# GEO-IASS/bn-pp

Hardware: NVIDIA B200
Metric: factor entries/sec (fused product+sum-out), VE PR on 2^28-entry tables (higher is better)
Workload: dtype f64

## Files before the change

### bnpp_b200/capi.py

```python
import ctypes
import os

_HERE = os.path.dirname(os.path.abspath(__file__))
LIB_PATH = os.path.join(_HERE, "libbnpp_b200.so")

c_u32p = ctypes.POINTER(ctypes.c_uint32)
c_i32p = ctypes.POINTER(ctypes.c_int32)
c_i64p = ctypes.POINTER(ctypes.c_int64)
c_u64p = ctypes.POINTER(ctypes.c_uint64)
c_f64p = ctypes.POINTER(ctypes.c_double)

EXPORTS = [
    "bnpp_version", "bnpp_ctx_create", "bnpp_ctx_destroy", "bnpp_ctx_sync", "bnpp_ctx_status", "bnpp_last_error",
    "bnpp_launch_count", "bnpp_last_launch", "bnpp_alloc", "bnpp_free", "bnpp_upload", "bnpp_download", "bnpp_fill",
    "bnpp_union_scope", "bnpp_scope_size", "bnpp_product_sum_out", "bnpp_product", "bnpp_sum_out", "bnpp_condition",
    "bnpp_normalize", "bnpp_reduce", "bnpp_fg_create", "bnpp_fg_destroy", "bnpp_fg_sweep", "bnpp_fg_update",
    "bnpp_fg_marginals", "bnpp_elim_order", "bnpp_order_width", "bnpp_ve_plan_create", "bnpp_ve_plan_destroy",
    "bnpp_ve_plan_info", "bnpp_ve_plan_run", "bnpp_ve_plan_run_batched", "bnpp_ve_plan_set_profiling",
    "bnpp_ve_plan_step_stats", "bnpp_ve_plan_step_kernel", "bnpp_ve_plan_set_fused", "bnpp_ve_plan_fused_info", "bnpp_ve_plan_fused_program", "bnpp_ve_plan_describe", "bnpp_ve_plan_set_segments", "bnpp_ve_plan_segments", "bnpp_ve_plan_segment_program", "bnpp_mar_plan_create", "bnpp_mar_plan_layout", "bnpp_pick_shard_vars",
    "bnpp_tuning_set", "bnpp_tuning_get", "bnpp_ve_plan_result_size", "bnpp_ve_plan_set_normalize",
    "bnpp_mar_plan_normalize", "bnpp_fg_reset", "bnpp_ve_plan_launches",
    "bnpp_sampler_create", "bnpp_sampler_destroy", "bnpp_sampler_logical", "bnpp_sampler_likelihood",
    "bnpp_product_max_out", "bnpp_mpe_plan_create", "bnpp_mpe_plan_run", "bnpp_mpe_plan_run_batched",
    "bnpp_elim_order_constrained", "bnpp_map_plan_create", "bnpp_mpe_plan_nvars", "bnpp_mpe_shard_select",
    "bnpp_ve_plan_windows",
]


def tuning_set(key, value):
    L = lib()
    L.bnpp_tuning_set.argtypes = [ctypes.c_char_p, ctypes.c_uint64]
    L.bnpp_tuning_get.argtypes = [ctypes.c_char_p, c_u64p]
    old = ctypes.c_uint64()
    if L.bnpp_tuning_get(key.encode(), ctypes.byref(old)) != 0 or L.bnpp_tuning_set(key.encode(), int(value)) != 0:
        raise BnppError(-1, "unknown tuning key %r" % key)
    return old.value


class Scope(ctypes.Structure):
    _fields_ = [("rank", ctypes.c_int32), ("var_id", c_u32p), ("card", c_u32p)]


class Operand(ctypes.Structure):
    _fields_ = [("data", ctypes.c_void_p), ("scope", Scope), ("stride", c_i64p)]


class BnppError(RuntimeError):
    def __init__(self, code, msg):
        super().__init__("bnpp_b200 error %d: %s" % (code, msg))
        self.code = code


_lib = None


def lib():
    global _lib
    if _lib is None:
        if not os.path.exists(LIB_PATH):
            raise RuntimeError("bnpp_b200: %s is not built (run `python -c 'import __graft_entry__ as g; g.build()'`); "
                               "there is no CPU fallback" % LIB_PATH)
        L = ctypes.CDLL(LIB_PATH)
        L.bnpp_last_error.restype = ctypes.c_char_p
        L.bnpp_last_error.argtypes = [ctypes.c_void_p]
        L.bnpp_launch_count.restype = ctypes.c_uint64
        L.bnpp_launch_count.argtypes = [ctypes.c_void_p]
        L.bnpp_scope_size.restype = ctypes.c_uint64
        L.bnpp_ctx_create.argtypes = [ctypes.c_int, ctypes.c_void_p, ctypes.POINTER(ctypes.c_void_p)]
        L.bnpp_ctx_destroy.argtypes = [ctypes.c_void_p]
        L.bnpp_ctx_sync.argtypes = [ctypes.c_void_p]
        L.bnpp_ctx_status.argtypes = [ctypes.c_void_p, c_u32p, ctypes.c_int]
        L.bnpp_last_launch.argtypes = [ctypes.c_void_p, ctypes.c_char_p, ctypes.c_size_t, c_u32p, c_u32p]
        L.bnpp_alloc.argtypes = [ctypes.c_void_p, ctypes.c_uint64, ctypes.POINTER(ctypes.c_void_p)]
        L.bnpp_free.argtypes = [ctypes.c_void_p, ctypes.c_void_p]
        L.bnpp_upload.argtypes = [ctypes.c_void_p, ctypes.c_void_p, ctypes.c_void_p, ctypes.c_uint64]
        L.bnpp_download.argtypes = [ctypes.c_void_p, ctypes.c_void_p, ctypes.c_void_p, ctypes.c_uint64]
        L.bnpp_fill.argtypes = [ctypes.c_void_p, ctypes.c_void_p, ctypes.c_uint64, ctypes.c_double]
        L.bnpp_union_scope.argtypes = [ctypes.POINTER(Scope), ctypes.POINTER(Scope), c_u32p, c_u32p]
        L.bnpp_scope_size.argtypes = [ctypes.POINTER(Scope)]
        L.bnpp_product_sum_out.argtypes = [ctypes.c_void_p, ctypes.c_int, ctypes.POINTER(Operand), ctypes.POINTER(Scope),
                                           ctypes.c_int64, ctypes.c_int, ctypes.c_void_p, ctypes.c_void_p]
        L.bnpp_product_max_out.argtypes = [ctypes.c_void_p, ctypes.c_int, ctypes.POINTER(Operand), ctypes.POINTER(Scope),
                                           ctypes.c_int64, ctypes.c_void_p, ctypes.c_void_p]
        L.bnpp_product.argtypes = [ctypes.c_void_p, ctypes.POINTER(Scope), ctypes.c_void_p, ctypes.POINTER(Scope),
                                   ctypes.c_void_p, ctypes.c_int, ctypes.c_void_p, ctypes.c_void_p]
        L.bnpp_sum_out.argtypes = [ctypes.c_void_p, ctypes.POINTER(Scope), ctypes.c_void_p, ctypes.c_uint32,
                                   ctypes.c_void_p, ctypes.c_void_p]
        L.bnpp_condition.argtypes = [ctypes.c_void_p, ctypes.POINTER(Scope), ctypes.c_void_p, ctypes.c_int, c_u32p, c_u32p,
                                     ctypes.c_void_p, ctypes.c_void_p]
        L.bnpp_normalize.argtypes = [ctypes.c_void_p, ctypes.c_uint64, ctypes.c_void_p, ctypes.c_void_p, ctypes.c_double,
                                     ctypes.c_void_p]
        L.bnpp_reduce.argtypes = [ctypes.c_void_p, ctypes.c_int, ctypes.c_uint64, ctypes.c_void_p, ctypes.c_double,
                                  ctypes.c_void_p]
        L.bnpp_fg_create.argtypes = [ctypes.c_void_p, ctypes.c_int, c_u32p, ctypes.c_int, c_i32p, c_u32p, c_u64p, c_f64p,
                                     ctypes.POINTER(ctypes.c_void_p)]
        L.bnpp_fg_destroy.argtypes = [ctypes.c_void_p]
        L.bnpp_fg_sweep.argtypes = [ctypes.c_void_p, c_f64p]
        L.bnpp_fg_update.argtypes = [ctypes.c_void_p, ctypes.c_uint32, ctypes.c_double, c_u32p]
        L.bnpp_fg_marginals.argtypes = [ctypes.c_void_p, c_f64p]
        _lib = L
    return _lib


def _u32(seq):
    arr = (ctypes.c_uint32 * max(1, len(seq)))(*[int(x) for x in seq])
    return arr


# ... 121 lines not shown
```

### bnpp_b200/csrc/chain.hpp

```cpp
#pragma once
#include <string>

#include "contract.hpp"

namespace bnpp {

constexpr int kChainMaxLevels = 4;
constexpr int kChainMaxSides = 2;
constexpr int kChainMaxAdd = 2;
constexpr int kChainTile = 16;
constexpr int kChainMaxUBits = 5;
constexpr int kChainMaxFields = 16;
constexpr uint32_t kChainDefaultDepth = 4;

__host__ __device__ constexpr uint32_t chain_chunk_items(int m) { return (m == 2 ? 2u : 1u) * kBlock; }

struct ChainSide {
    const double *p;
    uint32_t us[kChainMaxUBits];
    uint8_t nf;
    Field f[kChainMaxFields];
};

struct ChainLevel {
    uint8_t k;
    ChainSide s[kChainMaxSides];
};

struct ChainParams {
    const double *head;
    double *out;
    uint32_t n_items;
    uint8_t onf;
    Field of[kChainMaxFields];
    uint32_t os[4];
    ChainLevel lv[kChainMaxLevels];
};

const void *chain_kernel(int m, const int *add);
int chain_occupancy(const void *fn);
std::string chain_name(int m, const int *add);

}
```

### bnpp_b200/csrc/contract_chain.cu

```cuda
#include <cstdio>
#include <string>
#include <utility>

#include "chain.hpp"
#include "common.cuh"

namespace bnpp {

__device__ __forceinline__ uint32_t chain_fields(const Field *f, uint32_t nf, uint32_t r)
{
    uint32_t o = 0;
    for (uint32_t i = 0; i < nf; ++i) o += ((r >> f[i].sh) & f[i].mask) * f[i].mul;
    return o;
}

__device__ __forceinline__ uint32_t ubit_off(const uint32_t (&us)[kChainMaxUBits], int nbits, int u)
{
    uint32_t o = 0;
#pragma unroll
    for (int b = 0; b < kChainMaxUBits; ++b)
        if (b < nbits && ((u >> b) & 1)) o += us[b];
    return o;
}

template <int M, int J, int NB, int A, int KS>
__device__ __forceinline__ void chain_level_k(const ChainLevel &L, const uint32_t (&base)[kChainMaxSides],
                                              const double (&in)[kChainTile], double (&out)[kChainTile])
{
    constexpr int INB = M - J + NB;
    constexpr int UB = INB + A;
    constexpr int OUT = 1 << (UB - 1);
    constexpr int G = OUT < 4 ? OUT : (UB >= 5 ? 2 : 4);
    static_assert(INB <= 4 && UB - 1 <= 4 && UB <= kChainMaxUBits, "chain tile too large");
    const double *s0 = L.s[0].p + base[0];
    const double *s1 = L.s[1].p + base[1];
#pragma unroll
    for (int g = 0; g < OUT; g += G) {
        double a[2 * G], b[2 * G];
#pragma unroll
        for (int i = 0; i < 2 * G; ++i) {
            if (KS >= 1) a[i] = __ldg(s0 + ubit_off(L.s[0].us, UB, 2 * g + i));
            if (KS >= 2) b[i] = __ldg(s1 + ubit_off(L.s[1].us, UB, 2 * g + i));
        }
#pragma unroll
        for (int o = 0; o < G; ++o) {
            double p[2];
#pragma unroll
            for (int x = 0; x < 2; ++x) {
                const int i = 2 * o + x;
                const double h = in[(2 * g + i) & ((1 << INB) - 1)];
                p[x] = KS == 0 ? h : (KS == 1 ? __dmul_rn(h, a[i]) : __dmul_rn(__dmul_rn(a[i], b[i]), h));
            }
            out[g + o] = __dadd_rn(p[0], p[1]);
        }
    }
}

template <int M, int J, int NB, int A>
__device__ __forceinline__ void chain_level(const ChainLevel &L, const uint32_t (&base)[kChainMaxSides],
                                            const double (&in)[kChainTile], double (&out)[kChainTile])
{
    if (L.k == 0) chain_level_k<M, J, NB, A, 0>(L, base, in, out);
    else if (L.k == 1) chain_level_k<M, J, NB, A, 1>(L, base, in, out);
    else chain_level_k<M, J, NB, A, 2>(L, base, in, out);
}

template <int M, int A0, int A1, int A2, int A3>
__global__ void __launch_bounds__(kBlock) contract_chain(const __grid_constant__ ChainParams p)
{
    constexpr uint32_t CH = chain_chunk_items(M);
    constexpr int U = CH / kBlock;
    constexpr int NT = A0 + (M > 1 ? A1 : 0) + (M > 2 ? A2 : 0) + (M > 3 ? A3 : 0);
    uint32_t slo[U][M][kChainMaxSides], olo[U];
#pragma unroll
    for (int u = 0; u < U; ++u) {
        const uint32_t r = threadIdx.x + u * kBlock;
        olo[u] = chain_fields(p.of, p.onf, r);
#pragma unroll
        for (int j = 0; j < M; ++j)
#pragma unroll
            for (int q = 0; q < kChainMaxSides; ++q)
                slo[u][j][q] = q < p.lv[j].k ? chain_fields(p.lv[j].s[q].f, p.lv[j].s[q].nf, r) : 0u;
    }
    const uint32_t n_chunks = p.n_items / CH;
    for (uint32_t c = blockIdx.x; c < n_chunks; c += gridDim.x) {
        const uint32_t rb = c * CH;
        uint32_t shi[M][kChainMaxSides];
#pragma unroll
        for (int j = 0; j < M; ++j)
#pragma unroll
            for (int q = 0; q < kChainMaxSides; ++q)
                shi[j][q] = q < p.lv[j].k ? chain_fields(p.lv[j].s[q].f, p.lv[j].s[q].nf, rb) : 0u;
        const uint32_t ohi = chain_fields(p.of, p.onf, rb);
        double a[U][kChainTile], b[U][kChainTile];
#pragma unroll
        for (int u = 0; u < U; ++u) {
            const double *src = p.head + ((uint64_t)(rb + threadIdx.x + u * kBlock) << M);
#pragma unroll
            for (int i = 0; i < (1 << M); i += 4) {
                const double4_t v = ld4(src + i);
                a[u][i] = v.x; a[u][i + 1] = v.y; a[u][i + 2] = v.z; a[u][i + 3] = v.w;
            }
        }
#pragma unroll
        for (int u = 0; u < U; ++u) {
            uint32_t base[kChainMaxLevels][kChainMaxSides];
#pragma unroll
            for (int j = 0; j < M; ++j)
#pragma unroll
                for (int q = 0; q < kChainMaxSides; ++q) base[j][q] = shi[j][q] + slo[u][j][q];
            chain_level<M, 0, 0, A0>(p.lv[0], base[0], a[u], b[u]);
            if constexpr (M > 1) chain_level<M, 1, A0, A1>(p.lv[1], base[1], b[u], a[u]);
            if constexpr (M > 2) chain_level<M, 2, A0 + A1, A2>(p.lv[2], base[2], a[u], b[u]);
            if constexpr (M > 3) chain_level<M, 3, A0 + A1 + A2, A3>(p.lv[3], base[3], b[u], a[u]);
            double *o = p.out + (ohi + olo[u]);
#pragma unroll
            for (int i = 0; i < (1 << NT); ++i) {
                uint32_t off = 0;
#pragma unroll
                for (int bit = 0; bit < NT; ++bit)
                    if ((i >> bit) & 1) off += p.os[bit];
                if constexpr (M & 1) o[off] = b[u][i];
                else o[off] = a[u][i];
            }
        }
    }
}

namespace {

constexpr bool chain_shape_ok(int m, int a0, int a1, int a2, int a3)
{
    const int add[4] = {a0, a1, a2, a3};
    int nb = 0;
    for (int j = 0; j < 4; ++j) {
        if (j >= m) {
            if (add[j]) return false;
            continue;
        }
        const int inb = m - j + nb;
        const int outb = inb - 1 + add[j];
        if (inb > 4 || outb > 4) return false;
        nb += add[j];
    }
    return true;
}

constexpr int kChainCodes = 3 * 81;

template <int C>
constexpr const void *chain_entry()
{
    constexpr int m = C / 81 + 2, a0 = C % 3, a1 = C / 3 % 3, a2 = C / 9 % 3, a3 = C / 27 % 3;
    if constexpr (chain_shape_ok(m, a0, a1, a2, a3))
        return reinterpret_cast<const void *>(contract_chain<m, a0, a1, a2, a3>);
    else
        return nullptr;
}

template <int... C>
const void *chain_table(int code, std::integer_sequence<int, C...>)
{
    static const void *const table[] = {chain_entry<C>()...};
    return table[code];
}

}

const void *chain_kernel(int m, const int *add)
{
    if (m < 2 || m > kChainMaxLevels) return nullptr;
    int code = (m - 2) * 81, w = 1;
    for (int j = 0; j < kChainMaxLevels; ++j, w *= 3) {
        const int a = j < m ? add[j] : 0;
        if (a < 0 || a > kChainMaxAdd) return nullptr;
        code += a * w;
    }
    return chain_table(code, std::make_integer_sequence<int, kChainCodes>());
}

int chain_occupancy(const void *fn)
{
    int n = 0;
    if (cudaOccupancyMaxActiveBlocksPerMultiprocessor(&n, fn, kBlock, 0) != cudaSuccess) return 0;
    return n;
}

std::string chain_name(int m, const int *add)
{
    std::string s = "contract_chain<D=" + std::to_string(m) + ",add=";
    for (int j = 0; j < m; ++j) s += std::to_string(add[j]);
    return s + ">";
}

}
```

### bnpp_b200/csrc/ve.cu

```cuda
#include <algorithm>
#include <atomic>
#include <chrono>
#include <cstdio>
#include <cstdlib>
#include <cstring>
#include <map>
#include <memory>
#include <thread>
#include <vector>

#include "batched.hpp"
#include "chain.hpp"
#include "common.cuh"
#include "contract.hpp"
#include "elim_order.hpp"
#include "fused.hpp"

namespace bnpp {
int contract(bnpp_ctx *ctx, int k, const bnpp_operand *ops, const bnpp_scope *out_scope, int64_t elim_var, int divide,
             double *out_dev, double *z_dev, bool max_mode = false, uint8_t *arg_dev = nullptr);
int fill(bnpp_ctx *ctx, double *out, uint64_t n, double value);
int normalize_segments(bnpp_ctx *ctx, double *buf, const uint32_t *off_dev, const uint32_t *size_dev, int n);
int normalize_segments_batched(bnpp_ctx *ctx, double *buf, const uint32_t *off_dev, const uint32_t *size_dev, int n, uint32_t nb);
uint32_t chain_depth_knob();
// ... 1187 lines not shown
constexpr uint64_t kChainMaxSide = 1ull << 16;

int64_t factor_stride(const PlanFactor &pf, uint32_t v)
{
    int64_t dense = 1;
    for (size_t i = pf.var.size(); i-- > 0;) {
        const int64_t st = pf.stride.empty() ? dense : pf.stride[i];
        if (pf.var[i] == v) return st;
        dense *= pf.card[i];
    }
    return 0;
}

bool chain_fields(const PlanFactor &pf, const std::vector<uint32_t> &rest, Field *f, uint8_t &nf)
{
    nf = 0;
    for (size_t b = 0; b < rest.size();) {
        const int64_t st = factor_stride(pf, rest[b]);
        if (!st) { ++b; continue; }
        size_t len = 1;
        while (b + len < rest.size() && factor_stride(pf, rest[b + len]) == (st << len)) ++len;
        if (nf == kChainMaxFields || st > UINT32_MAX) return false;
        f[nf++] = Field{(uint32_t)((1ull << len) - 1), (uint32_t)st, (uint32_t)b};
        b += len;
    }
    return true;
}

bool chain_shape(const bnpp_ve_plan *pl, int head, const std::vector<int> &lv, bnpp_ve_plan::Window &w)
{
    const int m = (int)lv.size();
    const PlanFactor &H = pl->f[head];
    const int nh = (int)H.var.size();
    if (m < 2 || m > kChainMaxLevels || nh < m || !H.stride.empty()) return false;
    std::vector<uint32_t> rest;
    for (int b = nh - m - 1; b >= 0; --b) rest.push_back(H.var[b]);
    const uint64_t n_items = H.size >> m;
    if (n_items % chain_chunk_items(m) || n_items > UINT32_MAX) return false;
    w = bnpp_ve_plan::Window();
    w.m = m;
    w.head = head;
    memset(&w.p, 0, sizeof w.p);
    w.p.n_items = (uint32_t)n_items;
    std::vector<uint32_t> added;
    std::vector<int> sides_seen;
    int in = head, nb = 0;
    w.bytes = 8 * H.size;
    for (int j = 0; j < m; ++j) {
        const PlanStep &st = pl->steps[lv[j]];
        if (st.elim != (int64_t)H.var[nh - 1 - j] || st.out < 0) return false;
        std::vector<uint32_t> ub;
        for (int i = j; i < m; ++i) ub.push_back(H.var[nh - 1 - i]);
        ub.insert(ub.end(), added.begin(), added.end());
        ChainLevel &L = w.p.lv[j];
        int hpos = -1, k = 0;
        for (size_t q = 0; q < st.operands.size(); ++q) {
            const int id = st.operands[q];
            if (id == in && hpos < 0) { hpos = (int)q; continue; }
            if (k == kChainMaxSides) return false;
            w.side[j][k++] = id;
        }
        if (hpos < 0) return false;
        if (k == 2 && hpos != 2) return false;
        L.k = (uint8_t)k;
        int add = 0;
        for (int q = 0; q < k; ++q)
            for (uint32_t v : pl->f[w.side[j][q]].var)
                if (std::find(ub.begin(), ub.end(), v) == ub.end() && std::find(rest.begin(), rest.end(), v) == rest.end()) {
                    ub.push_back(v);
                    added.push_back(v);
                    ++add;
                }
        if (add > kChainMaxAdd) return false;
        const int inb = m - j + nb, outb = inb - 1 + add;
        if (inb > 4 || outb > 4 || (int)ub.size() != inb + add) return false;
        w.add[j] = add;
        nb += add;
        for (int q = 0; q < k; ++q) {
            const PlanFactor &S = pl->f[w.side[j][q]];
            for (size_t b = 0; b < ub.size(); ++b) {
                const int64_t sv = factor_stride(S, ub[b]);
                if (sv > UINT32_MAX) return false;
                L.s[q].us[b] = (uint32_t)sv;
            }
            if (!chain_fields(S, rest, L.s[q].f, L.s[q].nf)) return false;
            if (std::find(sides_seen.begin(), sides_seen.end(), w.side[j][q]) == sides_seen.end()) {
                sides_seen.push_back(w.side[j][q]);
                w.bytes += 8 * S.size;
            }
        }
        const PlanFactor &O = pl->f[st.out];
        if (O.var.size() != ub.size() - 1 + rest.size()) return false;
        w.entries += st.union_entries;
        in = st.out;
    }
    const PlanFactor &O = pl->f[in];
    if (O.size > UINT32_MAX || !O.stride.empty()) return false;
    for (size_t i = 0; i < added.size(); ++i) w.p.os[i] = (uint32_t)factor_stride(O, added[i]);
    if (!chain_fields(O, rest, w.p.of, w.p.onf)) return false;
    w.out = in;
    w.bytes += 8 * O.size;
    w.fn = chain_kernel(m, w.add);
    if (!w.fn) return false;
    w.name = chain_name(m, w.add);
    return true;
}

void set_launches(bnpp_ve_plan *pl)
{
    const size_t ns = pl->steps.size();
    if (pl->window_at.size() != ns) pl->window_at.assign(ns, -1);
    pl->launch_first.clear();
    uint64_t bytes = 0;
    for (size_t s = 0; s < ns; ++s) {
        pl->launch_first.push_back((int)s);
        if (pl->window_at[s] >= 0) {
            const auto &w = pl->windows[pl->window_at[s]];
            bytes += w.bytes;
            s = (size_t)w.b - 1;
        } else {
            bytes += pl->steps[s].bytes;
        }
    }
    pl->bytes = bytes;
}

void form_windows(bnpp_ve_plan *pl)
{
    if (pl->runs || pl->arena || pl->batch_runs || !pl->offtab_host.empty()) return;
    const size_t ns = pl->steps.size();
    pl->windows.clear();
    pl->window_at.assign(ns, -1);
    bool any_max = false;
    for (const PlanStep &st : pl->steps) any_max |= st.max;
    if (pl->is_mpe || pl->is_mar || any_max || pl->chain_depth < 2 || ns < 3) {
        set_launches(pl);
        return;
    }
    std::vector<int> producer(pl->f.size(), -1), nread(pl->f.size(), 0), reader(pl->f.size(), -1);
    for (size_t s = 0; s < ns; ++s) {
        const PlanStep &st = pl->steps[s];
        if (st.out >= 0) producer[st.out] = (int)s;
        std::vector<int> seen;
        for (int id : st.operands)
            if (std::find(seen.begin(), seen.end(), id) == seen.end()) {
                seen.push_back(id);
                nread[id]++;
                reader[id] = (int)s;
            }
    }
    auto binary = [&](const PlanStep &st) {
        for (int id : st.operands)
            for (uint32_t c : pl->f[id].card)
                if (c != 2) return false;
        return true;
    };
    auto link = [&](int s) {
        const PlanStep &a = pl->steps[s];
        if (a.out < 0 || a.want_z || nread[a.out] != 1 || pl->f[a.out].var.empty()) return -1;
        const int t = reader[a.out];
        const PlanStep &b = pl->steps[t];
        if (b.out < 0 || b.want_z || b.elim < 0 || b.union_entries < kChainMinUnion) return -1;
        if (pl->f[a.out].var.back() != (uint32_t)b.elim || !binary(a) || !binary(b)) return -1;
        for (int id : b.operands)
            if (id != a.out && pl->f[id].size > kChainMaxSide) return -1;
        return t;
// ... 731 lines not shown
    }
    *words = w.size();
    if (buf) {
        if (cap < w.size()) return BNPP_EINVAL;
        std::copy(w.begin(), w.end(), buf);
    }
    return BNPP_OK;
}

int bnpp_ve_plan_set_segments(bnpp_ve_plan *pl, int on, uint32_t max_steps)
{
    if (!pl) return BNPP_EINVAL;
    if (pl->is_mpe && on) return fail(pl->ctx, BNPP_EINVAL, "MPE plans run one launch per bucket (ve_tasks only sums)");
    pl->segments_mode = on != 0 ? 1 : 0;
    if (pl->graph_exec && pl->graph_groups != (on != 0)) {
        cudaGraphExecDestroy(pl->graph_exec);
        cudaGraphDestroy(pl->graph);
        pl->graph_exec = nullptr;
        pl->graph = nullptr;
    }
    if (on && (!pl->levels_built || max_steps != pl->segments_max_steps)) {
        pl->segments_max_steps = max_steps;
        build_levels(pl);
        form_windows(pl);
    }
    return BNPP_OK;
}

static int dump_program(const FusedProgram &fp, uint32_t *prog, uint64_t prog_cap, uint64_t *prog_words, uint32_t *offtab,
                        uint64_t tab_cap, uint64_t *tab_words)
{
    if (prog_words) *prog_words = fp.prog.size();
    if (tab_words) *tab_words = fp.offtab.size();
    if (prog) {
        if (prog_cap < fp.prog.size()) return BNPP_EINVAL;
        std::copy(fp.prog.begin(), fp.prog.end(), prog);
        for (auto &slot : fp.ptr_slots) {
            prog[slot.lo] = (uint32_t)slot.index;
            prog[slot.hi] = slot.kind == 0 ? 0xffffffffu : 0xfffffffeu;
        }
    }
    if (offtab) {
        if (tab_cap < fp.offtab.size()) return BNPP_EINVAL;
        std::copy(fp.offtab.begin(), fp.offtab.end(), offtab);
    }
    return BNPP_OK;
}

int bnpp_ve_plan_segments(bnpp_ve_plan *pl, uint32_t cap, uint32_t *n, uint32_t *first_step, uint32_t *end_step,
                          int32_t *lanes, uint32_t *arena_doubles)
{
    if (!pl || !n) return BNPP_EINVAL;
    if (!pl->segments_built) build_segments(pl);
    *n = (uint32_t)pl->segs.size();
    for (uint32_t i = 0; i < *n && i < cap; ++i) {
        if (first_step) first_step[i] = (uint32_t)pl->segs[i].a;
        if (end_step) end_step[i] = (uint32_t)pl->segs[i].b;
        if (lanes) lanes[i] = pl->segs[i].G;
        if (arena_doubles) arena_doubles[i] = pl->segs[i].prog.arena;
    }
    return BNPP_OK;
}

int bnpp_ve_plan_launches(bnpp_ve_plan *pl, uint64_t *launches, uint32_t *groups, uint32_t *levels)
{
    if (!pl) return BNPP_EINVAL;
    if (!pl->segments_built) build_segments(pl);
    uint64_t covered = 0;
    for (const auto &g : pl->groups) covered += (uint64_t)(g.b - g.a);
    for (const auto &w : pl->windows) covered += (uint64_t)(w.b - w.a - 1);
    if (launches) *launches = pl->steps.size() - covered + pl->groups.size();
    if (groups) *groups = (uint32_t)pl->groups.size();
    if (levels) *levels = pl->step_level.empty() ? 0u : (uint32_t)(*std::max_element(pl->step_level.begin(), pl->step_level.end()) + 1);
    return BNPP_OK;
}

int bnpp_ve_plan_windows(const bnpp_ve_plan *pl, uint32_t cap, uint32_t *n, uint32_t *first_step, uint32_t *n_steps)
{
    if (!pl || !n) return BNPP_EINVAL;
    *n = (uint32_t)pl->windows.size();
    for (uint32_t i = 0; i < *n && i < cap; ++i) {
        if (first_step) first_step[i] = (uint32_t)pl->windows[i].a;
        if (n_steps) n_steps[i] = (uint32_t)(pl->windows[i].b - pl->windows[i].a);
    }
    return BNPP_OK;
}

int bnpp_ve_plan_segment_program(bnpp_ve_plan *pl, uint32_t segment, uint32_t *prog, uint64_t prog_cap, uint64_t *prog_words,
                                 uint32_t *offtab, uint64_t tab_cap, uint64_t *tab_words)
{
    if (!pl) return BNPP_EINVAL;
    if (!pl->segments_built) build_segments(pl);
    if (segment >= pl->segs.size()) return BNPP_EINVAL;
    return dump_program(pl->segs[segment].prog, prog, prog_cap, prog_words, offtab, tab_cap, tab_words);
}

int bnpp_ve_plan_fused_program(bnpp_ve_plan *pl, uint32_t nb, uint32_t *prog, uint64_t prog_cap, uint64_t *prog_words,
                               uint32_t *offtab, uint64_t tab_cap, uint64_t *tab_words)
{
    if (!pl || nb == 0) return BNPP_EINVAL;
    const bool was_profiling = pl->profiling;
    pl->profiling = false;
    const int G = fused_pick(pl, nb);
    pl->profiling = was_profiling;
    if (prog_words) *prog_words = G ? pl->fused.prog.size() : 0;
    if (tab_words) *tab_words = G ? pl->fused.offtab.size() : 0;
    if (!G) return BNPP_OK;
    return dump_program(pl->fused, prog, prog_cap, prog_words, offtab, tab_cap, tab_words);
}

int bnpp_ve_plan_step_stats(bnpp_ve_plan *pl, uint64_t n, float *ms, uint64_t *bytes, uint64_t *entries, int32_t *k)
{
    if (!pl) return BNPP_EINVAL;
    const size_t ns = pl->steps.size();
    const bool win = !pl->windows.empty() && pl->window_at.size() == ns;
    auto launch_end = [&](size_t s) -> size_t { return win && pl->window_at[s] >= 0 ? (size_t)pl->windows[pl->window_at[s]].b : s + 1; };
    if (pl->profiling && !pl->ev.empty()) {
        BNPP_CUDA(pl->ctx, cudaEventSynchronize(pl->ev[ns]));
        pl->step_ms.clear();
        for (size_t s = 0; s < ns; s = launch_end(s)) {
            float t = 0.0f;
            BNPP_CUDA(pl->ctx, cudaEventElapsedTime(&t, pl->ev[s], pl->ev[launch_end(s)]));
            pl->step_ms.push_back(t);
        }
    }
    size_t row = 0;
    for (size_t s = 0; s < ns && row < n; s = launch_end(s), ++row) {
        const bool w = win && pl->window_at[s] >= 0;
        if (ms) ms[row] = row < pl->step_ms.size() ? pl->step_ms[row] : 0.0f;
        if (bytes) bytes[row] = w ? pl->windows[pl->window_at[s]].bytes : pl->steps[s].bytes;
        if (entries) entries[row] = w ? pl->windows[pl->window_at[s]].entries : pl->steps[s].union_entries;
        if (k) k[row] = (int32_t)pl->steps[s].operands.size();
    }
    return BNPP_OK;
}

int bnpp_ve_plan_step_kernel(const bnpp_ve_plan *pl, uint64_t step, char *name, size_t name_len)
{
    if (!pl || !name || !name_len) return BNPP_EINVAL;
    if (!pl->windows.empty()) step = step < pl->launch_first.size() ? (uint64_t)pl->launch_first[step] : UINT64_MAX;
    const std::string s = step < pl->step_kernel.size() ? pl->step_kernel[step] : std::string();
    strncpy(name, s.c_str(), name_len - 1);
    name[name_len - 1] = 0;
    return BNPP_OK;
}

static int run_dynamic(bnpp_ve_plan *pl, const std::vector<const double *> &ptr_in, double *result_dev, double *z_dev)
{
    bnpp_ctx *ctx = pl->ctx;
    std::vector<const double *> ptr = ptr_in;
    std::vector<double *> owned(pl->f.size(), nullptr);
    int rc = BNPP_OK;
    for (size_t s = 0; s < pl->steps.size() && rc == BNPP_OK; ++s) {
        const PlanStep &st = pl->steps[s];
        if (pl->profiling) cudaEventRecord(pl->ev[s], ctx->stream);
        bnpp_operand ops[kMaxK];
        for (size_t q = 0; q < st.operands.size(); ++q) {
            const PlanFactor &pf = pl->f[st.operands[q]];
            ops[q].data = ptr[st.operands[q]];
            ops[q].scope.rank = (int32_t)pf.var.size();
            ops[q].scope.var_id = pf.var.data();
            ops[q].scope.card = pf.card.data();
            ops[q].stride = pf.stride.empty() ? nullptr : pf.stride.data();
        }
        bnpp_scope os;
        double *dst;
// ... 740 lines not shown
```

### include/bnpp_b200.h

```cpp
#ifndef BNPP_B200_H_
#define BNPP_B200_H_

#include <stddef.h>
#include <stdint.h>

#ifdef __cplusplus
extern "C" {
#endif

#define BNPP_OK        0
#define BNPP_EINVAL   -1
#define BNPP_ECUDA    -2
#define BNPP_ERANK    -3
#define BNPP_ETOOBIG  -4
#define BNPP_ENOMEM   -5

#define BNPP_MAX_RANK      64
#define BNPP_MAX_AXES      32
#define BNPP_MAX_OPERANDS   6

#define BNPP_STATUS_ZERO_DIVISOR 1u
#define BNPP_STATUS_BAD_EVIDENCE 2u

typedef struct bnpp_ctx bnpp_ctx;
// ... 23 lines not shown
int bnpp_tuning_get(const char *key, uint64_t *value);

int bnpp_alloc(bnpp_ctx *ctx, uint64_t n_doubles, double **dptr);
int bnpp_free(bnpp_ctx *ctx, double *dptr);
int bnpp_upload(bnpp_ctx *ctx, double *dst_dev, const double *src_host, uint64_t n);
int bnpp_download(bnpp_ctx *ctx, double *dst_host, const double *src_dev, uint64_t n);
int bnpp_fill(bnpp_ctx *ctx, double *dst_dev, uint64_t n, double value);

int bnpp_union_scope(const bnpp_scope *a, const bnpp_scope *b, uint32_t *out_var_id, uint32_t *out_card);
uint64_t bnpp_scope_size(const bnpp_scope *s);

int bnpp_product_sum_out(bnpp_ctx *ctx, int k, const bnpp_operand *operands,
                         const bnpp_scope *out_scope, int64_t elim_var, int divide,
                         double *out_dev, double *z_dev);

int bnpp_product_max_out(bnpp_ctx *ctx, int k, const bnpp_operand *operands, const bnpp_scope *out_scope,
                         int64_t elim_var, double *out_dev, uint8_t *argmax_dev);

int bnpp_product(bnpp_ctx *ctx, const bnpp_scope *sa, const double *a_dev,
                 const bnpp_scope *sb, const double *b_dev, int divide,
                 double *out_dev, double *z_dev);
int bnpp_sum_out(bnpp_ctx *ctx, const bnpp_scope *s, const double *in_dev, uint32_t var,
                 double *out_dev, double *z_dev);
int bnpp_condition(bnpp_ctx *ctx, const bnpp_scope *s, const double *in_dev,
                   int n_ev, const uint32_t *ev_var, const uint32_t *ev_val,
                   double *out_dev, double *z_dev);
int bnpp_normalize(bnpp_ctx *ctx, uint64_t n, const double *in_dev, const double *z_dev, double z_host,
                   double *out_dev);
int bnpp_reduce(bnpp_ctx *ctx, int op, uint64_t n, const double *in_dev, double init, double *result_dev);

int bnpp_elim_order(int nvars, const uint32_t *card, int nfac, const bnpp_scope *scopes, int n_obs,
                    const uint32_t *obs_var, int n_vars_to_order, const uint32_t *vars, int heuristic,
                    uint32_t *order_out, uint32_t *n_order_out, uint32_t *width_out);
int bnpp_elim_order_constrained(int nvars, const uint32_t *card, int nfac, const bnpp_scope *scopes, int n_obs,
                                const uint32_t *obs_var, int n_first, const uint32_t *first, int n_last,
                                const uint32_t *last, int heuristic, uint32_t *order_out, uint32_t *n_order_out,
                                uint32_t *width_out);
int bnpp_pick_shard_vars(int nfac, const bnpp_scope *scopes, int n_order, const uint32_t *order, int g, uint32_t *out);
int bnpp_order_width(int nvars, const uint32_t *card, int nfac, const bnpp_scope *scopes, int n_order,
                     const uint32_t *order, uint32_t *width_out);

typedef struct bnpp_ve_plan bnpp_ve_plan;
int bnpp_ve_plan_create(bnpp_ctx *ctx, int nfac, const bnpp_scope *scopes, int n_obs, const uint32_t *obs_var,
                        int n_order, const uint32_t *order, bnpp_ve_plan **out);
int bnpp_ve_plan_destroy(bnpp_ve_plan *plan);
int bnpp_ve_plan_info(const bnpp_ve_plan *plan, int32_t *result_rank, uint32_t *result_var, uint32_t *result_card,
                      uint64_t *n_launches, uint64_t *union_entries, uint64_t *algorithmic_bytes,
                      uint64_t *peak_bytes, uint64_t *max_step_entries);
int bnpp_ve_plan_run(bnpp_ve_plan *plan, const double *const *tables_dev, const uint32_t *obs_val,
                     double *result_dev, double *z_dev);
int bnpp_mpe_plan_create(bnpp_ctx *ctx, int nvars, const uint32_t *card, int nfac, const bnpp_scope *scopes,
                         int n_obs, const uint32_t *obs_var, int n_order, const uint32_t *order, bnpp_ve_plan **out);
#define BNPP_ASSIGN_SUMMED 0xFFFFFFFFu
int bnpp_map_plan_create(bnpp_ctx *ctx, int nvars, const uint32_t *card, int nfac, const bnpp_scope *scopes,
                         int n_obs, const uint32_t *obs_var, int n_map, const uint32_t *map_var, int n_order,
                         const uint32_t *order, bnpp_ve_plan **out);
int bnpp_mpe_plan_run(bnpp_ve_plan *plan, const double *const *tables_dev, const uint32_t *obs_val,
                      double *value_dev, uint32_t *assignment_dev);
int bnpp_mpe_plan_nvars(const bnpp_ve_plan *plan, uint32_t *nvars);
int bnpp_mpe_shard_select(bnpp_ctx *ctx, uint32_t nranks, uint32_t nvars, const uint32_t *records_dev, double *value_dev,
                          uint32_t *assignment_dev);
int bnpp_mpe_plan_run_batched(bnpp_ve_plan *plan, const double *const *tables_dev, uint32_t nb, uint32_t n_obs,
                              const uint8_t *ev_dev, double *value_dev, uint8_t *assignment_dev);
int bnpp_ve_plan_result_size(const bnpp_ve_plan *plan, uint64_t *n);
int bnpp_mar_plan_create(bnpp_ctx *ctx, int nvars, const uint32_t *card, int nfac, const bnpp_scope *scopes, int n_obs,
                         const uint32_t *obs_var, int n_order, const uint32_t *order, bnpp_ve_plan **out);
int bnpp_mar_plan_layout(const bnpp_ve_plan *plan, int nvars, uint32_t *off, uint32_t *size, uint64_t *total);
int bnpp_ve_plan_set_normalize(bnpp_ve_plan *plan, int on);
int bnpp_mar_plan_normalize(bnpp_ve_plan *plan, double *result_dev);

int bnpp_ve_plan_run_batched(bnpp_ve_plan *plan, const double *const *tables_dev, uint32_t nb, uint32_t n_obs,
                             const uint8_t *ev_dev, double *result_dev);
int bnpp_ve_plan_set_fused(bnpp_ve_plan *plan, int on);
int bnpp_ve_plan_fused_info(bnpp_ve_plan *plan, uint32_t nb, int32_t *lanes_per_set, uint32_t *arena_doubles,
                            uint32_t *n_steps);
int bnpp_ve_plan_fused_program(bnpp_ve_plan *plan, uint32_t nb, uint32_t *prog, uint64_t prog_cap, uint64_t *prog_words,
                               uint32_t *offtab, uint64_t tab_cap, uint64_t *tab_words);
int bnpp_ve_plan_describe(const bnpp_ve_plan *plan, uint64_t *buf, uint64_t cap, uint64_t *words);
int bnpp_ve_plan_set_segments(bnpp_ve_plan *plan, int on, uint32_t max_steps);
int bnpp_ve_plan_segments(bnpp_ve_plan *plan, uint32_t cap, uint32_t *n, uint32_t *first_step, uint32_t *end_step,
                          int32_t *lanes, uint32_t *arena_doubles);
int bnpp_ve_plan_launches(bnpp_ve_plan *plan, uint64_t *launches, uint32_t *groups, uint32_t *levels);
int bnpp_ve_plan_windows(const bnpp_ve_plan *plan, uint32_t cap, uint32_t *n, uint32_t *first_step, uint32_t *n_steps);
int bnpp_ve_plan_segment_program(bnpp_ve_plan *plan, uint32_t segment, uint32_t *prog, uint64_t prog_cap, uint64_t *prog_words,
                                 uint32_t *offtab, uint64_t tab_cap, uint64_t *tab_words);
int bnpp_ve_plan_set_profiling(bnpp_ve_plan *plan, int on);
int bnpp_ve_plan_step_stats(bnpp_ve_plan *plan, uint64_t n, float *ms, uint64_t *bytes, uint64_t *entries, int32_t *k);
int bnpp_ve_plan_step_kernel(const bnpp_ve_plan *plan, uint64_t step, char *name, size_t name_len);

typedef struct bnpp_fg bnpp_fg;
int bnpp_fg_create(bnpp_ctx *ctx, int nvars, const uint32_t *card, int nfac,
                   const int32_t *foff, const uint32_t *fscope,
                   const uint64_t *toff, const double *ftab_host, bnpp_fg **out);
int bnpp_fg_destroy(bnpp_fg *fg);
int bnpp_fg_sweep(bnpp_fg *fg, double *maxerror_host);
int bnpp_fg_update(bnpp_fg *fg, uint32_t max_sweeps, double epsilon, uint32_t *sweeps);
int bnpp_fg_reset(bnpp_fg *fg);
int bnpp_fg_marginals(bnpp_fg *fg, double *out_host);

typedef struct bnpp_sampler bnpp_sampler;
int bnpp_sampler_create(bnpp_ctx *ctx, int nvars, const uint32_t *card, const bnpp_scope *scopes, const uint32_t *order,
                        const double *const *tables_dev, bnpp_sampler **out);
int bnpp_sampler_destroy(bnpp_sampler *s);
int bnpp_sampler_logical(bnpp_sampler *s, int n_ev, const uint32_t *ev_var, const uint32_t *ev_val, uint64_t n_samples,
                         uint64_t seed, uint64_t *hits);
int bnpp_sampler_likelihood(bnpp_sampler *s, int n_ev, const uint32_t *ev_var, const uint32_t *ev_val, double u_bound,
                            double n_star, uint64_t batch, uint64_t max_samples, uint64_t seed, double *n_sum, uint64_t *m);

#ifdef __cplusplus
}
#endif
#endif
```

Measured before the change: 1378 billion.

## Specialize chain levels on side dependency masks to load only distinct factor entries

Records for each chain level a bitmask of which tile bits the side factors actually depend on, and dispatches to compile-time specializations that load and multiply only the distinct factor entries instead of one per tile point. Side-table offsets are now computed per level per item instead of being precomputed and held in registers, and k==0 levels become plain pairwise adds. Each chain shape also gets a per-shape minimum-blocks launch bound. The aim is fewer gather loads and multiplies plus lower register pressure for higher occupancy, at the cost of more template instantiations, larger code and extra per-item index arithmetic. A query API for window level metadata is also added.

```diff
diff --git a/bnpp_b200/capi.py b/bnpp_b200/capi.py
--- a/bnpp_b200/capi.py
+++ b/bnpp_b200/capi.py
@@ -23,7 +23,7 @@
     "bnpp_sampler_create", "bnpp_sampler_destroy", "bnpp_sampler_logical", "bnpp_sampler_likelihood",
     "bnpp_product_max_out", "bnpp_mpe_plan_create", "bnpp_mpe_plan_run", "bnpp_mpe_plan_run_batched",
     "bnpp_elim_order_constrained", "bnpp_map_plan_create", "bnpp_mpe_plan_nvars", "bnpp_mpe_shard_select",
-    "bnpp_ve_plan_windows",
+    "bnpp_ve_plan_windows", "bnpp_ve_plan_window_levels",
 ]
 
 
diff --git a/bnpp_b200/csrc/chain.hpp b/bnpp_b200/csrc/chain.hpp
--- a/bnpp_b200/csrc/chain.hpp
+++ b/bnpp_b200/csrc/chain.hpp
@@ -24,6 +24,7 @@
 
 struct ChainLevel {
     uint8_t k;
+    uint8_t dep;
     ChainSide s[kChainMaxSides];
 };
 
diff --git a/bnpp_b200/csrc/contract_chain.cu b/bnpp_b200/csrc/contract_chain.cu
--- a/bnpp_b200/csrc/contract_chain.cu
+++ b/bnpp_b200/csrc/contract_chain.cu
@@ -23,96 +23,144 @@
     return o;
 }
 
+__host__ __device__ constexpr int chain_batch(int ub) { return ub >= 5 ? 4 : (ub >= 3 ? 8 : 1 << ub); }
+
+__host__ __device__ constexpr int chain_dep(int inb, int a, int mid) { return 1 | mid << 1 | ((1 << a) - 1) << inb; }
+__host__ __device__ constexpr int dep_point(int dep, int d)
+{
+    int u = 0;
+    for (int b = 0, i = 0; b < kChainMaxUBits; ++b)
+        if ((dep >> b) & 1) u |= ((d >> i++) & 1) << b;
+    return u;
+}
+__host__ __device__ constexpr int dep_index(int dep, int u)
+{
+    int d = 0;
+    for (int b = 0, i = 0; b < kChainMaxUBits; ++b)
+        if ((dep >> b) & 1) d |= ((u >> b) & 1) << i++;
+    return d;
+}
+
+template <int M, int J, int NB, int A, int KS, int DEP>
+__device__ __forceinline__ void chain_level_dep(const ChainLevel &L, const uint32_t (&base)[kChainMaxSides],
+                                                const double (&in)[kChainTile], double (&out)[kChainTile])
+{
+    constexpr int INB = M - J + NB, UB = INB + A, OUT = 1 << (UB - 1);
+    constexpr int ND = dep_index(DEP, DEP) + 1;
+    constexpr int VB = ND < chain_batch(UB) ? ND : chain_batch(UB);
+    const double *s0 = L.s[0].p + base[0];
+    const double *s1 = L.s[1].p + base[1];
+#pragma unroll
+    for (int d0 = 0; d0 < ND; d0 += VB) {
+        double v[VB], w[VB];
+#pragma unroll
+        for (int i = 0; i < VB; ++i) {
+            v[i] = __ldg(s0 + ubit_off(L.s[0].us, UB, dep_point(DEP, d0 + i)));
+            if (KS == 2) w[i] = __ldg(s1 + ubit_off(L.s[1].us, UB, dep_point(DEP, d0 + i)));
+        }
+        if (KS == 2) {
+#pragma unroll
+            for (int i = 0; i < VB; ++i) v[i] = __dmul_rn(v[i], w[i]);
+        }
+#pragma unroll
+        for (int o = 0; o < OUT; ++o) {
+            const int d = dep_index(DEP, 2 * o) - d0;
+            if (d < 0 || d >= VB) continue;
+            const double h0 = in[(2 * o) & ((1 << INB) - 1)], h1 = in[(2 * o + 1) & ((1 << INB) - 1)];
+            out[o] = __dadd_rn(__dmul_rn(v[d], h0), __dmul_rn(v[d + 1], h1));
+        }
+    }
+}
+
+template <int M, int J, int NB, int A, int KS, int... MID>
+__device__ __forceinline__ bool chain_level_masked(const ChainLevel &L, const uint32_t (&base)[kChainMaxSides],
+                                                   const double (&in)[kChainTile], double (&out)[kChainTile],
+                                                   std::integer_sequence<int, MID...>)
+{
+    constexpr int INB = M - J + NB;
+    return ((L.dep == chain_dep(INB, A, MID) &&
+             (chain_level_dep<M, J, NB, A, KS, chain_dep(INB, A, MID)>(L, base, in, out), true)) || ...);
+}
+
 template <int M, int J, int NB, int A, int KS>
 __device__ __forceinline__ void chain_level_k(const ChainLevel &L, const uint32_t (&base)[kChainMaxSides],
                                               const double (&in)[kChainTile], double (&out)[kChainTile])
 {
+    constexpr int INB = M - J + NB, UB = INB + A;
+    constexpr int NMASKED = UB >= 4 ? (1 << (INB - 1)) - 1 : 0;
+    if (!chain_level_masked<M, J, NB, A, KS>(L, base, in, out, std::make_integer_sequence<int, NMASKED>()))
+        chain_level_dep<M, J, NB, A, KS, (1 << UB) - 1>(L, base, in, out);
+}
+
+template <int M, int J, int NB, int A>
+__device__ __forceinline__ void chain_level(const ChainLevel &L, uint32_t r, const double (&in)[kChainTile],
+                                            double (&out)[kChainTile])
+{
     constexpr int INB = M - J + NB;
-    constexpr int UB = INB + A;
-    constexpr int OUT = 1 << (UB - 1);
-    constexpr int G = OUT < 4 ? OUT : (UB >= 5 ? 2 : 4);
-    static_assert(INB <= 4 && UB - 1 <= 4 && UB <= kChainMaxUBits, "chain tile too large");
-    const double *s0 = L.s[0].p + base[0];
-    const double *s1 = L.s[1].p + base[1];
-#pragma unroll
-    for (int g = 0; g < OUT; g += G) {
-        double a[2 * G], b[2 * G];
-#pragma unroll
-        for (int i = 0; i < 2 * G; ++i) {
-            if (KS >= 1) a[i] = __ldg(s0 + ubit_off(L.s[0].us, UB, 2 * g + i));
-            if (KS >= 2) b[i] = __ldg(s1 + ubit_off(L.s[1].us, UB, 2 * g + i));
-        }
-#pragma unroll
-        for (int o = 0; o < G; ++o) {
-            double p[2];
-#pragma unroll
-            for (int x = 0; x < 2; ++x) {
-                const int i = 2 * o + x;
-                const double h = in[(2 * g + i) & ((1 << INB) - 1)];
-                p[x] = KS == 0 ? h : (KS == 1 ? __dmul_rn(h, a[i]) : __dmul_rn(__dmul_rn(a[i], b[i]), h));
-            }
-            out[g + o] = __dadd_rn(p[0], p[1]);
-        }
-    }
-}
-
-template <int M, int J, int NB, int A>
-__device__ __forceinline__ void chain_level(const ChainLevel &L, const uint32_t (&base)[kChainMaxSides],
-                                            const double (&in)[kChainTile], double (&out)[kChainTile])
-{
-    if (L.k == 0) chain_level_k<M, J, NB, A, 0>(L, base, in, out);
-    else if (L.k == 1) chain_level_k<M, J, NB, A, 1>(L, base, in, out);
-    else chain_level_k<M, J, NB, A, 2>(L, base, in, out);
+    static_assert(INB <= 4 && INB + A - 1 <= 4 && INB + A <= kChainMaxUBits, "chain tile too large");
+    uint32_t base[kChainMaxSides];
+#pragma unroll
+    for (int q = 0; q < kChainMaxSides; ++q) base[q] = q < L.k ? chain_fields(L.s[q].f, L.s[q].nf, r) : 0u;
+    if (L.k == 0) {
+#pragma unroll
+        for (int o = 0; o < (1 << (INB - 1)); ++o) out[o] = __dadd_rn(in[2 * o], in[2 * o + 1]);
+    } else if (L.k == 1) {
+        chain_level_k<M, J, NB, A, 1>(L, base, in, out);
+    } else {
+        chain_level_k<M, J, NB, A, 2>(L, base, in, out);
+    }
+}
+
+constexpr unsigned char kChainMinBlocks[3 * 81] = {
+    6, 5, 4, 6, 4, 3, 5, 4, 2, 0, 0, 0, 0, 0, 0, 0, 0, 0, 0, 0, 0, 0, 0, 0, 0, 0, 0,
+    0, 0, 0, 0, 0, 0, 0, 0, 0, 0, 0, 0, 0, 0, 0, 0, 0, 0, 0, 0, 0, 0, 0, 0, 0, 0, 0,
+    0, 0, 0, 0, 0, 0, 0, 0, 0, 0, 0, 0, 0, 0, 0, 0, 0, 0, 0, 0, 0, 0, 0, 0, 0, 0, 0,
+    6, 4, 4, 6, 4, 2, 6, 2, 0, 6, 5, 2, 6, 3, 1, 4, 2, 0, 6, 4, 4, 5, 3, 0, 3, 0, 0,
+    0, 0, 0, 0, 0, 0, 0, 0, 0, 0, 0, 0, 0, 0, 0, 0, 0, 0, 0, 0, 0, 0, 0, 0, 0, 0, 0,
+    0, 0, 0, 0, 0, 0, 0, 0, 0, 0, 0, 0, 0, 0, 0, 0, 0, 0, 0, 0, 0, 0, 0, 0, 0, 0, 0,
+    4, 2, 0, 4, 2, 0, 3, 0, 0, 4, 2, 0, 4, 2, 0, 2, 0, 0, 4, 2, 0, 2, 0, 0, 0, 0, 0,
+    4, 2, 0, 4, 2, 0, 3, 0, 0, 4, 2, 0, 4, 2, 0, 2, 0, 0, 4, 1, 0, 2, 0, 0, 0, 0, 0,
+    4, 2, 0, 4, 2, 0, 3, 0, 0, 4, 2, 0, 3, 0, 0, 0, 0, 0, 3, 0, 0, 0, 0, 0, 0, 0, 0,
+};
+
+constexpr int chain_min_blocks(int m, int a0, int a1, int a2, int a3)
+{
+    return kChainMinBlocks[(m - 2) * 81 + a0 + 3 * a1 + 9 * a2 + 27 * a3];
 }
 
 template <int M, int A0, int A1, int A2, int A3>
-__global__ void __launch_bounds__(kBlock) contract_chain(const __grid_constant__ ChainParams p)
+__global__ void __launch_bounds__(kBlock, chain_min_blocks(M, A0, A1, A2, A3)) contract_chain(const __grid_constant__ ChainParams p)
 {
     constexpr uint32_t CH = chain_chunk_items(M);
     constexpr int U = CH / kBlock;
     constexpr int NT = A0 + (M > 1 ? A1 : 0) + (M > 2 ? A2 : 0) + (M > 3 ? A3 : 0);
-    uint32_t slo[U][M][kChainMaxSides], olo[U];
-#pragma unroll
-    for (int u = 0; u < U; ++u) {
-        const uint32_t r = threadIdx.x + u * kBlock;
-        olo[u] = chain_fields(p.of, p.onf, r);
-#pragma unroll
-        for (int j = 0; j < M; ++j)
-#pragma unroll
-            for (int q = 0; q < kChainMaxSides; ++q)
-                slo[u][j][q] = q < p.lv[j].k ? chain_fields(p.lv[j].s[q].f, p.lv[j].s[q].nf, r) : 0u;
-    }
+    uint32_t olo[U];
+#pragma unroll
+    for (int u = 0; u < U; ++u) olo[u] = chain_fields(p.of, p.onf, threadIdx.x + u * kBlock);
     const uint32_t n_chunks = p.n_items / CH;
     for (uint32_t c = blockIdx.x; c < n_chunks; c += gridDim.x) {
         const uint32_t rb = c * CH;
-        uint32_t shi[M][kChainMaxSides];
-#pragma unroll
-        for (int j = 0; j < M; ++j)
-#pragma unroll
-            for (int q = 0; q < kChainMaxSides; ++q)
-                shi[j][q] = q < p.lv[j].k ? chain_fields(p.lv[j].s[q].f, p.lv[j].s[q].nf, rb) : 0u;
         const uint32_t ohi = chain_fields(p.of, p.onf, rb);
-        double a[U][kChainTile], b[U][kChainTile];
+        double h[U][1 << M];
 #pragma unroll
         for (int u = 0; u < U; ++u) {
             const double *src = p.head + ((uint64_t)(rb + threadIdx.x + u * kBlock) << M);
 #pragma unroll
             for (int i = 0; i < (1 << M); i += 4) {
                 const double4_t v = ld4(src + i);
-                a[u][i] = v.x; a[u][i + 1] = v.y; a[u][i + 2] = v.z; a[u][i + 3] = v.w;
+                h[u][i] = v.x; h[u][i + 1] = v.y; h[u][i + 2] = v.z; h[u][i + 3] = v.w;
             }
         }
 #pragma unroll
         for (int u = 0; u < U; ++u) {
-            uint32_t base[kChainMaxLevels][kChainMaxSides];
-#pragma unroll
-            for (int j = 0; j < M; ++j)
-#pragma unroll
-                for (int q = 0; q < kChainMaxSides; ++q) base[j][q] = shi[j][q] + slo[u][j][q];
-            chain_level<M, 0, 0, A0>(p.lv[0], base[0], a[u], b[u]);
-            if constexpr (M > 1) chain_level<M, 1, A0, A1>(p.lv[1], base[1], b[u], a[u]);
-            if constexpr (M > 2) chain_level<M, 2, A0 + A1, A2>(p.lv[2], base[2], a[u], b[u]);
-            if constexpr (M > 3) chain_level<M, 3, A0 + A1 + A2, A3>(p.lv[3], base[3], b[u], a[u]);
+            double a[kChainTile], b[kChainTile];
+#pragma unroll
+            for (int i = 0; i < (1 << M); ++i) a[i] = h[u][i];
+            const uint32_t r = rb + threadIdx.x + u * kBlock;
+            chain_level<M, 0, 0, A0>(p.lv[0], r, a, b);
+            if constexpr (M > 1) chain_level<M, 1, A0, A1>(p.lv[1], r, b, a);
+            if constexpr (M > 2) chain_level<M, 2, A0 + A1, A2>(p.lv[2], r, a, b);
+            if constexpr (M > 3) chain_level<M, 3, A0 + A1 + A2, A3>(p.lv[3], r, b, a);
             double *o = p.out + (ohi + olo[u]);
 #pragma unroll
             for (int i = 0; i < (1 << NT); ++i) {
@@ -120,8 +168,8 @@
 #pragma unroll
                 for (int bit = 0; bit < NT; ++bit)
                     if ((i >> bit) & 1) off += p.os[bit];
-                if constexpr (M & 1) o[off] = b[u][i];
-                else o[off] = a[u][i];
+                if constexpr (M & 1) o[off] = b[i];
+                else o[off] = a[i];
             }
         }
     }
@@ -152,8 +200,10 @@
 constexpr const void *chain_entry()
 {
     constexpr int m = C / 81 + 2, a0 = C % 3, a1 = C / 3 % 3, a2 = C / 9 % 3, a3 = C / 27 % 3;
-    if constexpr (chain_shape_ok(m, a0, a1, a2, a3))
+    if constexpr (chain_shape_ok(m, a0, a1, a2, a3)) {
+        static_assert(kChainMinBlocks[C] > 0, "a chain shape without its CTAs per SM");
         return reinterpret_cast<const void *>(contract_chain<m, a0, a1, a2, a3>);
+    }
     else
         return nullptr;
 }
diff --git a/bnpp_b200/csrc/ve.cu b/bnpp_b200/csrc/ve.cu
--- a/bnpp_b200/csrc/ve.cu
+++ b/bnpp_b200/csrc/ve.cu
@@ -1293,6 +1293,7 @@
                 const int64_t sv = factor_stride(S, ub[b]);
                 if (sv > UINT32_MAX) return false;
                 L.s[q].us[b] = (uint32_t)sv;
+                if (sv) L.dep |= (uint8_t)(1u << b);
             }
             if (!chain_fields(S, rest, L.s[q].f, L.s[q].nf)) return false;
             if (std::find(sides_seen.begin(), sides_seen.end(), w.side[j][q]) == sides_seen.end()) {
@@ -2190,6 +2191,29 @@
     for (uint32_t i = 0; i < *n && i < cap; ++i) {
         if (first_step) first_step[i] = (uint32_t)pl->windows[i].a;
         if (n_steps) n_steps[i] = (uint32_t)(pl->windows[i].b - pl->windows[i].a);
+    }
+    return BNPP_OK;
+}
+
+int bnpp_ve_plan_window_levels(const bnpp_ve_plan *pl, uint32_t window, uint32_t *m, uint32_t *k, uint32_t *ubits,
+                               uint32_t *side_mask, uint32_t *dep)
+{
+    if (!pl || window >= pl->windows.size()) return BNPP_EINVAL;
+    const auto &w = pl->windows[window];
+    if (m) *m = (uint32_t)w.m;
+    int nb = 0;
+    for (int j = 0; j < w.m; ++j) {
+        const ChainLevel &L = w.p.lv[j];
+        if (k) k[j] = L.k;
+        if (dep) dep[j] = L.dep;
+        if (ubits) ubits[j] = (uint32_t)(w.m - j + nb + w.add[j]);
+        nb += w.add[j];
+        for (int q = 0; q < kChainMaxSides; ++q) {
+            uint32_t mask = 0;
+            for (int b = 0; b < kChainMaxUBits && q < L.k; ++b)
+                if (L.s[q].us[b]) mask |= 1u << b;
+            if (side_mask) side_mask[2 * j + q] = mask;
+        }
     }
     return BNPP_OK;
 }
diff --git a/include/bnpp_b200.h b/include/bnpp_b200.h
--- a/include/bnpp_b200.h
+++ b/include/bnpp_b200.h
@@ -129,6 +129,8 @@
                           int32_t *lanes, uint32_t *arena_doubles);
 int bnpp_ve_plan_launches(bnpp_ve_plan *plan, uint64_t *launches, uint32_t *groups, uint32_t *levels);
 int bnpp_ve_plan_windows(const bnpp_ve_plan *plan, uint32_t cap, uint32_t *n, uint32_t *first_step, uint32_t *n_steps);
+int bnpp_ve_plan_window_levels(const bnpp_ve_plan *plan, uint32_t window, uint32_t *m, uint32_t *k, uint32_t *ubits,
+                               uint32_t *side_mask, uint32_t *dep);
 int bnpp_ve_plan_segment_program(bnpp_ve_plan *plan, uint32_t segment, uint32_t *prog, uint64_t prog_cap, uint64_t *prog_words,
                                  uint32_t *offtab, uint64_t tab_cap, uint64_t *tab_words);
 int bnpp_ve_plan_set_profiling(bnpp_ve_plan *plan, int on);
```

Result: faster. 1488 billion, median of 6 (+8.0%).
